# zrc0622/HIRL4UCAV

Measured on AMD Instinct MI355X. Metric: env steps/sec (whole node) + HIRL update steps/sec at 4096 envs/GPU, higher is better.
Workload: dtype f32

## Files before the change

hirl4ucav_amd/csrc/hx_wgrad.hip:

```cpp
#include <cmath>

#include "hx_update.h"

using namespace hxnn;
using namespace hxu;

namespace {

struct WgJobC {
    const float* net; float* grad;
    float* ws0; float* ws1;
    float* mom; float* var; float* target; uint16_t* w2b; float* w2f;
    uint32_t cfg;
    int32_t rows0, rows1;
    float slope, w_given, warm, inv_batch;
    float b1, b2, eps, step_size, bc2_sqrt, tau;
    uint32_t pad_;
    const int* soft_count; float* wstate; float* losses;
    uint16_t* w2tb; uint16_t* tgt_w2b;
    float* count_out;
};
static_assert(sizeof(WgJobC) == 176, "WgJobC layout");
struct WgArgsC {
    WgJobC job[2];
    int has_pre, pre_batch;
    SampleDev pre;
};

struct AdamElem {
    float p, m, v, t;
    __device__ __forceinline__ void fetch(const WgJob& J, unsigned idx) {
        p = J.p[idx];
        m = J.mom[idx];
        v = J.var[idx];
        t = J.target ? J.target[idx] : 0.0f;
    }
    __device__ __forceinline__ void apply(const WgJob& J, const WgAdam& a, unsigned idx, float g) {
        adam_update(p, m, v, g, a.b1, a.b2, a.eps, a.step_size, a.bc2_sqrt);
        J.p[idx] = p;
        J.mom[idx] = m;
        J.var[idx] = v;
        if (J.target) {
            t = polyak_update(t, p, a.tau);
            J.target[idx] = t;
        }
    }
};

constexpr int kWgTilesPerBlock = 2 * (H2 / 16);
constexpr int kWgCols = 16;
constexpr int kWgVecWgs = H2 / kWgCols;
constexpr int kWgL1Wgs = H1 / kWgCols;
constexpr int kWgRG = kWide / kWgCols;
constexpr int kWgPerJob = kWgTilesPerBlock + kWgVecWgs + kWgL1Wgs;
constexpr int kWgRowChunk = 256;

constexpr int kRedP = 21;
__device__ __forceinline__ float sum_groups(const float* p, int half) {
    constexpr int N = kWgRG / 2;
    float v[N];
#pragma unroll
    for (int g = 0; g < N; ++g) v[g] = p[(2 * g + half) * kWgCols * kRedP];
#pragma unroll
    for (int w = 1; w < N; w *= 2)
#pragma unroll
        for (int g = 0; g < N; g += 2 * w) v[g] += v[g + w];
    const float other = __int_as_float(__builtin_amdgcn_mov_dpp(__float_as_int(v[0]), 0xB1, 0xf, 0xf, true));
    return half ? other + v[0] : v[0] + other;
}

__device__ __forceinline__ void expand_wg(const WgJobC& c, WgJob& J, WgArgs& A) {
    J.net = c.net; J.grad = c.grad; J.m = mlp_of(c.cfg & 1023u);
    J.nslots = (int)((c.cfg >> 10) & 3u);
    J.wmode[0] = (int)((c.cfg >> 12) & 3u); J.wmode[1] = (int)((c.cfg >> 14) & 3u);
    J.ws[0] = carve_slot(c.ws0, c.rows0); J.ws[1] = carve_slot(c.ws1, c.rows1);
    J.rows[0] = c.rows0; J.rows[1] = c.rows1;
    J.p = const_cast<float*>(c.net); J.mom = c.mom; J.var = c.var; J.target = c.target; J.w2b = c.w2b; J.w2f = c.w2f;
    J.w2tb = c.w2tb; J.tgt_w2b = c.tgt_w2b; J.w2b_x9 = (int)((c.cfg >> 20) & 1u);
    A.slope = c.slope; A.w_kind = (int)((c.cfg >> 16) & 3u); A.w_given = c.w_given; A.warm = c.warm; A.inv_batch = c.inv_batch;
    A.soft_count = c.soft_count; A.wstate = c.wstate;
    A.ad.b1 = c.b1; A.ad.b2 = c.b2; A.ad.eps = c.eps; A.ad.step_size = c.step_size; A.ad.bc2_sqrt = c.bc2_sqrt; A.ad.tau = c.tau;
    A.ad.finish_actor = (int)((c.cfg >> 18) & 1u); A.ad.use_bc = (int)((c.cfg >> 19) & 1u);
    A.ad.losses = c.losses; A.ad.wstate = c.wstate;
    A.count_out = c.count_out;
    A.ad.alpha_state = nullptr; A.ad.target_entropy = 0.0f; A.ad.alpha_step_size = 0.0f;
    if ((c.cfg >> 21) & 1u) {
        A.ad.alpha_state = c.wstate; A.ad.target_entropy = c.w_given; A.ad.alpha_step_size = c.warm;
        A.ad.wstate = nullptr; A.wstate = nullptr; A.w_given = 0.0f; A.warm = 0.0f;
    }
}
inline WgJobC pack_wg(const WgJob& J, const WgArgs& A) {
    WgJobC c{};
    c.net = J.net; c.grad = J.grad; c.ws0 = J.ws[0].x; c.ws1 = J.nslots > 1 ? J.ws[1].x : J.ws[0].x;
    c.mom = J.mom; c.var = J.var; c.target = J.target; c.w2b = J.w2b; c.w2f = J.w2f; c.w2tb = J.w2tb; c.tgt_w2b = J.tgt_w2b;
    c.cfg = mlp_bits(J.m) | ((uint32_t)J.nslots << 10) | ((uint32_t)J.wmode[0] << 12) | ((uint32_t)J.wmode[1] << 14) | ((uint32_t)A.w_kind << 16) |
            ((uint32_t)(A.ad.finish_actor ? 1 : 0) << 18) | ((uint32_t)(A.ad.use_bc ? 1 : 0) << 19) | ((uint32_t)(J.w2b_x9 ? 1 : 0) << 20) |
            ((uint32_t)(A.ad.alpha_state ? 1 : 0) << 21);
    c.rows0 = J.rows[0]; c.rows1 = J.nslots > 1 ? J.rows[1] : J.rows[0];
    c.slope = A.slope; c.w_given = A.w_given; c.warm = A.warm; c.inv_batch = A.inv_batch;
    c.b1 = A.ad.b1; c.b2 = A.ad.b2; c.eps = A.ad.eps; c.step_size = A.ad.step_size; c.bc2_sqrt = A.ad.bc2_sqrt; c.tau = A.ad.tau;
    c.soft_count = A.soft_count; c.wstate = const_cast<float*>(A.wstate); c.losses = A.ad.losses; c.count_out = A.count_out;
    if (A.ad.alpha_state) { c.wstate = A.ad.alpha_state; c.w_given = A.ad.target_entropy; c.warm = A.ad.alpha_step_size; }
    return c;
}

#ifdef HX_STAMPS_L1
#define STAMP_L1() STAMP()
#else
#define STAMP_L1()
#endif
template <bool ADAM, bool RELU, bool BF16 = false>
__global__ __launch_bounds__(kWide) void wgrad_kernel(WgArgsC AC) {
    __shared__ __attribute__((aligned(16))) float lds[kWgRowChunk * XP + kWgRowChunk * 12 + kWgRG * kWgCols * kRedP];
    float* xs = lds;
    float* rinfo = lds + kWgRowChunk * XP;
    float* red = rinfo + kWgRowChunk * 12;

    {
        static_assert(sizeof(lds) >= (4 * kFusedSlots + 2 * kFusedBatchMax) * 4, "predraw_wg's tables fit");
        if (AC.has_pre && blockIdx.x >= kWgPerJob) {
            if (blockIdx.x == kWgPerJob && blockIdx.y == 0) predraw_wg(AC.pre, AC.pre_batch, lds);
            return;
        }
    }
    const int j = blockIdx.y, b = blockIdx.x;
    WgJob J;
    WgArgs A;
    expand_wg(AC.job[j], J, A);
    const int tid = threadIdx.x, wave = tid >> 6, lane = tid & 63;
    const float slope = A.slope;
    STAMP_DECL;
    STAMP();
    const float w = effective_w(A.w_kind, A.w_given, A.warm, A.inv_batch, A.soft_count, A.wstate);
    float scale[2];
#pragma unroll
    for (int s = 0; s < 2; ++s) scale[s] = J.wmode[s] == 0 ? 1.0f : (J.wmode[s] == 1 ? 1.0f - w : w);
#ifdef HX_STAMPS
    asm volatile("" ::"v"(w));
    STAMP();
#endif
    if (A.count_out && blockIdx.x == 0 && blockIdx.y == 0 && tid == 0) *A.count_out = A.soft_count ? (float)*A.soft_count : 0.0f;
    if (ADAM && A.ad.finish_actor && blockIdx.x == 0 && blockIdx.y == 0 && tid == 0) {
        if (A.ad.use_bc) {
            A.ad.losses[1] = A.ad.losses[2] * w + A.ad.losses[3] * (1.0f - w);
            A.ad.losses[5] = w;
            *A.ad.wstate = w;
        } else {
            A.ad.losses[1] = A.ad.losses[3];
        }
    }
    if (ADAM && A.ad.alpha_state && blockIdx.x == 0 && blockIdx.y == 0 && tid == 0)
        sac_alpha_step(A.ad.alpha_state, A.ad.losses, A.ad.losses[4], A.ad.target_entropy, A.ad.b1, A.ad.b2, A.ad.eps, A.ad.alpha_step_size, A.ad.bc2_sqrt);

    if (b < kWgTilesPerBlock) {
        const int n0 = (b >> 1) * 16, k0 = (b & 1) * (H1 / 2) + (wave & 7) * 16, half = wave >> 3;
        const int r = lane & 15, g = lane >> 4;
        v4f acc = {0.f, 0.f, 0.f, 0.f};
        #pragma unroll
        for (int s = 0; s < 2; ++s) if (s < J.nslots) {
            const float sc = scale[s];
            const float* dz = J.ws[s].dz2;
            const float* h1 = J.ws[s].h1;
            const unsigned dzo = (unsigned)(n0 + r), h1o = (unsigned)(k0 + r);
            const int rows = J.rows[s];
            const int hr = ((rows + 7) >> 3) << 2;
            const int rbeg = half * hr, rend = min(rows, rbeg + hr);
            if constexpr (BF16) {
                v4f accs = {0.f, 0.f, 0.f, 0.f};
                for (int c0 = rbeg; c0 < rend; c0 += 64) {
                    float av[2][8], hv[2][8];
#pragma unroll
                    for (int m = 0; m < 2; ++m)
#pragma unroll
                        for (int j = 0; j < 8; ++j) {
                            const int row = c0 + 32 * m + 8 * g + j;
                            const unsigned rc = (unsigned)(row < rows ? row : rows - 1);
                            av[m][j] = dz[rc * (unsigned)H2 + dzo];
                            hv[m][j] = h1[rc * (unsigned)H1 + h1o];
                        }
#pragma unroll
                    for (int m = 0; m < 2; ++m) {
#pragma unroll
                        for (int j = 0; j < 8; ++j)
                            if (c0 + 32 * m + 8 * g + j >= rend) av[m][j] = 0.0f;
                        accs = mfma16_bf16(pack8_bf16(av[m]), pack8_bf16(hv[m]), accs);
                    }
                }
#pragma unroll
                for (int q = 0; q < 4; ++q) acc[q] = __builtin_fmaf(sc, accs[q], acc[q]);
            } else {
                for (int c0 = rbeg; c0 < rend; c0 += 64) {
                    float av[16], hv[16];
#pragma unroll
                    for (int i = 0; i < 16; ++i) {
                        const int row = c0 + 4 * i + g;
                        const unsigned rc = (unsigned)(row < rows ? row : rows - 1);
                        av[i] = dz[rc * (unsigned)H2 + dzo];
                        hv[i] = h1[rc * (unsigned)H1 + h1o];
                    }
#pragma unroll
                    for (int i = 0; i < 16; ++i) acc = mfma16(av[i] * (c0 + 4 * i + g < rend ? sc : 0.0f), hv[i], acc);
                }
            }
        }
        STAMP();
        const int q0 = 2 * half;
        AdamElem ae[2];
        if (ADAM) {
#pragma unroll
            for (int q = 0; q < 2; ++q) ae[q].fetch(J, J.m.W2() + (n0 + 4 * g + q0 + q) * H1 + k0 + r);
        }
        float2* xch = reinterpret_cast<float2*>(red);
        xch[((wave & 7) * 2 + half) * 64 + lane] = half ? make_float2(acc[0], acc[1]) : make_float2(acc[2], acc[3]);
        __syncthreads();
        const float2 got = xch[((wave & 7) * 2 + (half ^ 1)) * 64 + lane];
        const float fin[2] = {half ? got.x + acc[2] : acc[0] + got.x, half ? got.y + acc[3] : acc[1] + got.y};
        float* out = J.grad + J.m.W2();
#pragma unroll
        for (int q = 0; q < 2; ++q) out[(unsigned)((n0 + 4 * g + q0 + q) * H1 + k0 + r)] = fin[q];
        if (ADAM) {
#pragma unroll
            for (int q = 0; q < 2; ++q) {
                const int idx = J.m.W2() + (n0 + 4 * g + q0 + q) * H1 + k0 + r;
                ae[q].apply(J, A.ad, idx, fin[q]);
                if (J.w2b) {
                    const uint32_t ix = w2_image_index((uint32_t)(n0 + 4 * g + q0 + q), (uint32_t)(k0 + r));
                    uint16_t hi, mid, lo;
                    split3_bf16(ae[q].p, hi, mid, lo);
                    J.w2b[ix] = hi;
                    if (J.w2b_x9) { J.w2b[kImgElems + ix] = mid; J.w2b[2 * kImgElems + ix] = lo; }
                }
                if (J.w2f) J.w2f[w2f_image_index((uint32_t)(n0 + 4 * g + q0 + q), (uint32_t)(k0 + r))] = ae[q].p;
                if (J.w2tb) {
                    const __bf16 bv = (__bf16)ae[q].p;
                    J.w2tb[w2t_image_index((uint32_t)(k0 + r), (uint32_t)(n0 + 4 * g + q0 + q))] = __builtin_bit_cast(uint16_t, bv);
                }
                if (J.target && J.tgt_w2b) {
                    const __bf16 bv = (__bf16)ae[q].t;
                    J.tgt_w2b[w2_image_index((uint32_t)(n0 + 4 * g + q0 + q), (uint32_t)(k0 + r))] = __builtin_bit_cast(uint16_t, bv);
                }
            }
        }
        STAMP();
        STAMP_FLUSH(32, blockIdx.x == 0 && blockIdx.y == 0 && tid == 0);
        SPAN_LOG(HX_SPAN_WGRAD);
        return;
    }
    const int cl = lane & (kWgCols - 1);
    const int rg = tid / kWgCols;
    const int ohalf = tid & 1, oitem = (tid >> 1) / kWgCols, ocol = (tid >> 1) % kWgCols;
    if (b < kWgTilesPerBlock + kWgVecWgs) {
        constexpr int RP = 12;
        const int vb = b - kWgTilesPerBlock;
        const int n = vb * kWgCols + cl;
        const float g2 = J.net[J.m.g2() + n], be2 = J.net[J.m.be2() + n];
        float w3[OW];
#pragma unroll
        for (int jj = 0; jj < OW; ++jj) w3[jj] = jj < J.m.out ? J.net[J.m.W3() + jj * H2 + n] : 0.0f;
        float db2 = 0.f, dg = 0.f, dbe = 0.f, dw3[OW] = {}, db3 = 0.f;
        const int on = vb * kWgCols + ocol;
        const unsigned vidx = (unsigned)(oitem == 0 ? J.m.b2() + on : oitem == 1 ? J.m.g2() + on : oitem == 2 ? J.m.be2() + on : J.m.W3() + (oitem - 3) * H2 + on);
        const bool vlive = oitem < 3 + J.m.out;
        const bool b3live = vb == 0 && oitem == 3 + OW && ocol < J.m.out;
        const unsigned b3idx = (unsigned)(J.m.b3() + (ocol < J.m.out ? ocol : 0));
        AdamElem vae;
        bool vae_pending = ADAM && (vlive || b3live) && ohalf == 0;
        #pragma unroll
        for (int s = 0; s < 2; ++s) if (s < J.nslots) {
            const Slot& S = J.ws[s];
            const float sc = scale[s];
            for (int c0 = 0; c0 < J.rows[s]; c0 += kWgRowChunk) {
                const int nr = min(kWgRowChunk, J.rows[s] - c0);
                float zv[4], dv[4];
#pragma unroll
                for (int i = 0; i < 4; ++i) if (kWgRG * i < nr) {
                    const int r = rg + kWgRG * i;
                    const unsigned o = (unsigned)(c0 + (r < nr ? r : nr - 1)) * (unsigned)H2 + (unsigned)n;
                    zv[i] = S.z2[o];
                    dv[i] = S.dz2[o];
                }
                static_assert(kWgRowChunk <= kWide, "staging: one row per thread");
                const int er = tid < nr ? tid : 0;
                v2f st2v;
                v4f d4, d5;
                if (__builtin_amdgcn_readfirstlane(tid) < nr) {
                    st2v = *reinterpret_cast<const v2f*>(S.st2 + (size_t)(c0 + er) * 2);
                    d4 = *reinterpret_cast<const v4f*>(S.dout + (size_t)(c0 + er) * OW);
                    d5 = *reinterpret_cast<const v4f*>(S.dout + (size_t)(c0 + er) * OW + 4);
                }
                if (vae_pending) {
                    vae.fetch(J, b3live ? b3idx : vidx);
                    vae_pending = false;
                }
                __syncthreads();
                if (tid < nr) {
                    float4* r4 = reinterpret_cast<float4*>(rinfo + tid * RP);
                    r4[0] = make_float4(st2v[0], st2v[1], d4[0], d4[1]);
                    r4[1] = make_float4(d4[2], d4[3], d5[0], d5[1]);
                    r4[2] = make_float4(d5[2], d5[3], 0.0f, 0.0f);
                }
                __syncthreads();
                for (int rb0 = 0; rb0 < nr; rb0 += kWgRG * 4) {
                    const int rb = rg + rb0;
                    if (rb0 != 0) {
#pragma unroll
                        for (int i = 0; i < 4; ++i) if (rb0 + kWgRG * i < nr) {
                            const int r = rb + kWgRG * i;
                            const unsigned o = (unsigned)(c0 + (r < nr ? r : nr - 1)) * (unsigned)H2 + (unsigned)n;
                            zv[i] = S.z2[o];
                            dv[i] = S.dz2[o];
                        }
                    }
#pragma unroll
                    for (int i = 0; i < 4; ++i) {
                        const int r = rb + kWgRG * i;
                        if (r < nr) {
                            float ri[RP];
                            {
                                const float4* r4 = reinterpret_cast<const float4*>(rinfo + r * RP);
                                const float4 a = r4[0], b4 = r4[1], c4 = r4[2];
                                ri[0] = a.x; ri[1] = a.y; ri[2] = a.z; ri[3] = a.w; ri[4] = b4.x; ri[5] = b4.y; ri[6] = b4.z; ri[7] = b4.w;
                                ri[8] = c4.x; ri[9] = c4.y; ri[10] = c4.z; ri[11] = c4.w;
                            }
                            const float xh = (zv[i] - ri[0]) * ri[1];
                            const float y = g2 * xh + be2;
                            float dh2 = (ri[2] * w3[0] + ri[3] * w3[1]) + (ri[4] * w3[2] + ri[5] * w3[3]);
                            if (J.m.out > 4) dh2 += (ri[6] * w3[4] + ri[7] * w3[5]) + (ri[8] * w3[6] + ri[9] * w3[7]);
                            const float dy = act_bwd<RELU>(dh2, y, slope);
                            const float h2 = act_f<RELU>(y, slope);
                            db2 += sc * dv[i];
                            dbe += sc * dy;
                            dg += sc * dy * xh;
#pragma unroll
                            for (int jj = 0; jj < OW; ++jj) dw3[jj] += sc * ri[2 + jj] * h2;
                            if (vb == 0 && cl < J.m.out) db3 += sc * rinfo[r * RP + 2 + cl];
                        }
                    }
                }
            }
        }
        STAMP();
        float* my = red + (rg * kWgCols + cl) * kRedP;
        my[0] = db2; my[1] = dg; my[2] = dbe;
#pragma unroll
        for (int jj = 0; jj < OW; ++jj) my[3 + jj] = dw3[jj];
        my[3 + OW] = db3;
        __syncthreads();
        if (vlive || b3live) {
            float v = sum_groups(red + ocol * kRedP + oitem, ohalf);
            if ((oitem == 1 || oitem == 2) && J.m.no_ln) v = 0.0f;
            const unsigned idx = b3live ? b3idx : vidx;
            if (ohalf == 0) {
                J.grad[idx] = v;
                if (ADAM) vae.apply(J, A.ad, idx, v);
            }
        }
        STAMP();
        STAMP_FLUSH(40, b == kWgTilesPerBlock && j == 0 && tid == 0);
        SPAN_LOG(HX_SPAN_WGRAD);
        return;
    }
    {
        const int kb = (b - kWgTilesPerBlock - kWgVecWgs) * kWgCols;
        const int k = kb + cl;
        const int in = J.m.in;
        const float g1 = J.net[J.m.g1() + k], be1 = J.net[J.m.be1() + k];
        STAMP_L1();
        float db1 = 0.f, dg = 0.f, dbe = 0.f, dw1[17];
#pragma unroll
        for (int i = 0; i < 17; ++i) dw1[i] = 0.f;
        const int ok = kb + ocol;
        const unsigned lidx = (unsigned)(oitem == 0 ? J.m.b1() + ok : oitem == 1 ? J.m.g1() + ok : oitem == 2 ? J.m.be1() + ok : J.m.W1() + ok * in + (oitem - 3));
        const bool llive = oitem < 3 + in;
        AdamElem lae;
        bool lae_pending = ADAM && llive && ohalf == 0;
        #pragma unroll
        for (int s = 0; s < 2; ++s) if (s < J.nslots) {
            const Slot& S = J.ws[s];
            const float sc = scale[s];
            for (int c0 = 0; c0 < J.rows[s]; c0 += kWgRowChunk) {
                const int nr = min(kWgRowChunk, J.rows[s] - c0);
                float zv[4], dv[4];
#pragma unroll
                for (int i = 0; i < 4; ++i) if (kWgRG * i < nr) {
                    const int r = rg + kWgRG * i;
                    const unsigned o = (unsigned)(c0 + (r < nr ? r : nr - 1)) * (unsigned)H1 + (unsigned)k;
                    zv[i] = S.z1[o];
                    dv[i] = S.dh1[o];
                }
                STAMP_L1();
                static_assert(kWgRowChunk * XP <= 5 * kWide && kWgRowChunk <= kWide && kColWgB == 8, "staging: five words + one row per thread");
                const int w0 = __builtin_amdgcn_readfirstlane(tid);
                float xst[5];
#pragma unroll
                for (int q = 0; q < 5; ++q) {
                    const int e = tid + q * kWide;
                    if (w0 + q * kWide < nr * XP) xst[q] = S.x[(size_t)c0 * XP + (e < nr * XP ? e : 0)];
                }
                STAMP_L1();
                const int er = tid < nr ? tid : 0;
                v2f st1v;
                v4f l0, l1, l2, l3;
                if (w0 < nr) {
                    st1v = *reinterpret_cast<const v2f*>(S.st1 + (size_t)(c0 + er) * 2);
                    const v4f* lp4 = reinterpret_cast<const v4f*>(S.lnp + (size_t)(c0 + er) * (2 * kColWgB));
                    l0 = lp4[0]; l1 = lp4[1]; l2 = lp4[2]; l3 = lp4[3];
                }
                STAMP_L1();
                if (lae_pending) {
                    lae.fetch(J, lidx);
                    lae_pending = false;
                }
                STAMP_L1();
                __syncthreads();
                STAMP_L1();
#pragma unroll
                for (int q = 0; q < 5; ++q) {
                    const int e = tid + q * kWide;
                    if (e < nr * XP) xs[e] = xst[q];
                }
                if (tid < nr) {
                    const float s1 = ((l0[0] + l0[2]) + (l1[0] + l1[2])) + ((l2[0] + l2[2]) + (l3[0] + l3[2]));
                    const float s2 = ((l0[1] + l0[3]) + (l1[1] + l1[3])) + ((l2[1] + l2[3]) + (l3[1] + l3[3]));
                    *reinterpret_cast<float4*>(rinfo + tid * 8) = make_float4(st1v[0], st1v[1], s1 * (1.0f / H1), s2 * (1.0f / H1));
                }
                __syncthreads();
                STAMP_L1();
                for (int rb0 = 0; rb0 < nr; rb0 += kWgRG * 4) {
                    const int rb = rg + rb0;
                    if (rb0 != 0) {
#pragma unroll
                        for (int i = 0; i < 4; ++i) if (rb0 + kWgRG * i < nr) {
                            const int r = rb + kWgRG * i;
                            const unsigned o = (unsigned)(c0 + (r < nr ? r : nr - 1)) * (unsigned)H1 + (unsigned)k;
                            zv[i] = S.z1[o];
                            dv[i] = S.dh1[o];
                        }
                    }
#pragma unroll
                    for (int i = 0; i < 4; ++i) {
                        const int r = rb + kWgRG * i;
                        if (r < nr) {
                            const float4 ri = *reinterpret_cast<const float4*>(rinfo + r * 8);
                            const float xh = (zv[i] - ri.x) * ri.y;
                            const float dy = act_bwd<RELU>(dv[i], g1 * xh + be1, slope);
                            const float dz = sc * (ri.y * (dy * g1 - ri.z - xh * ri.w));
                            db1 += dz;
                            dbe += sc * dy;
                            dg += sc * dy * xh;
                            const float4* xr4 = reinterpret_cast<const float4*>(xs + r * XP);
#pragma unroll
                            for (int q = 0; q < 4; ++q) {
                                const float4 x4 = xr4[q];
                                dw1[4 * q] += dz * x4.x; dw1[4 * q + 1] += dz * x4.y; dw1[4 * q + 2] += dz * x4.z; dw1[4 * q + 3] += dz * x4.w;
                            }
                            dw1[16] += dz * xs[r * XP + 16];
                        }
                    }
                }
            }
        }
        STAMP_L1();
        float* my = red + (rg * kWgCols + cl) * kRedP;
        my[0] = db1; my[1] = dg; my[2] = dbe;
#pragma unroll
        for (int i = 0; i < 17; ++i) my[3 + i] = dw1[i];
        STAMP_L1();
        __syncthreads();
        STAMP_L1();
        if (llive) {
            float v = sum_groups(red + ocol * kRedP + oitem, ohalf);
            if ((oitem == 1 || oitem == 2) && J.m.no_ln) v = 0.0f;
#ifdef HX_STAMPS
            asm volatile("" ::"v"(v));
            STAMP_L1();
#endif
            if (ohalf == 0) {
                J.grad[lidx] = v;
                if (ADAM) lae.apply(J, A.ad, lidx, v);
            }
        }
        STAMP_L1();
        STAMP_FLUSH(48, b == kWgTilesPerBlock + kWgVecWgs && j == 0 && tid == 0);
        SPAN_LOG(HX_SPAN_WGRAD);
    }
}

__device__ __forceinline__ float adam_w(const AdamArgs& A) {
    if (A.countf && A.w_kind == 1) {
        const float w = *A.countf * A.inv_batch + A.warm;
        return w > 1.0f ? 1.0f : w;
    }
    return effective_w(A.w_kind, A.w_given, A.warm, A.inv_batch, A.soft_count, A.wstate);
}

__global__ __launch_bounds__(kThreads) void adam_kernel(AdamArgs A) {
    if (A.guard && __hip_atomic_load(A.guard, __ATOMIC_RELAXED, __HIP_MEMORY_SCOPE_SYSTEM) != 0u) return;
    if (A.alpha_state && blockIdx.x == 0 && threadIdx.x == 0)
        sac_alpha_step(A.alpha_state, A.losses, A.losses[4], A.target_entropy, A.b1, A.b2, A.eps, A.alpha_step_size, A.bc2_sqrt);
    const float wmix = A.g2 ? adam_w(A) : 0.0f;
    if (A.finish_actor && blockIdx.x == 0 && threadIdx.x == 0) {
        if (A.use_bc) {
            const float w = adam_w(A);
            A.losses[1] = A.losses[2] * w + A.losses[3] * (1.0f - w);
            A.losses[5] = w;
            *A.wstate = w;
        } else {
            A.losses[1] = A.losses[3];
        }
    }
    const int i = (blockIdx.x * kThreads + threadIdx.x) * 4;
    if (i >= A.n) return;
    if (i + 4 <= A.n) {
        float4 g4 = *reinterpret_cast<const float4*>(A.g + i);
        if (A.g2) {
            const float4 b4 = *reinterpret_cast<const float4*>(A.g2 + i);
            g4.x = wmix * b4.x + (1.0f - wmix) * g4.x;
            g4.y = wmix * b4.y + (1.0f - wmix) * g4.y;
            g4.z = wmix * b4.z + (1.0f - wmix) * g4.z;
            g4.w = wmix * b4.w + (1.0f - wmix) * g4.w;
        }
        adam_step4(A, i, make_float4(g4.x * A.gscale, g4.y * A.gscale, g4.z * A.gscale, g4.w * A.gscale));
        return;
    }
    for (int c = 0; c < A.n - i; ++c) {
        float pv = A.p[i + c], mv = A.m[i + c], vv = A.v[i + c];
        const float gv = A.g2 ? wmix * A.g2[i + c] + (1.0f - wmix) * A.g[i + c] : A.g[i + c];
        adam_update(pv, mv, vv, gv * A.gscale, A.b1, A.b2, A.eps, A.step_size, A.bc2_sqrt);
        A.p[i + c] = pv; A.m[i + c] = mv; A.v[i + c] = vv;
        if (A.target) A.target[i + c] = polyak_update(A.target[i + c], pv, A.tau);
    }
}

__global__ __launch_bounds__(kThreads) void polyak_kernel(float* target, const float* source, int n, float tau, float* target2 = nullptr,
                                                          const float* source2 = nullptr, int n2 = 0, const uint32_t* guard = nullptr) {
    if (guard && *guard != 0u) return;
    const int nb1 = (n / 4 + kThreads) / kThreads;
    int blk = blockIdx.x;
    if (blk >= nb1) {
        blk -= nb1; target = target2; source = source2; n = n2;
    }
    const int i = (blk * kThreads + threadIdx.x) * 4;
    if (i >= n) return;
    if (i + 4 <= n) {
        float4 t4 = *reinterpret_cast<const float4*>(target + i);
        const float4 s4 = *reinterpret_cast<const float4*>(source + i);
        t4.x = polyak_update(t4.x, s4.x, tau);
        t4.y = polyak_update(t4.y, s4.y, tau);
        t4.z = polyak_update(t4.z, s4.z, tau);
        t4.w = polyak_update(t4.w, s4.w, tau);
        *reinterpret_cast<float4*>(target + i) = t4;
        return;
    }
    for (int c = 0; c < n - i; ++c) target[i + c] = polyak_update(target[i + c], source[i + c], tau);
}

}

namespace hxu {

void launch_wg(const WgArgs& W, bool adam, hipStream_t st) {
    WgArgsC C{};
    for (int j = 0; j < W.njobs; ++j) C.job[j] = pack_wg(W.job[j], W);
    const bool pre = W.predraw != nullptr;
    C.has_pre = pre ? 1 : 0;
    if (pre) { C.pre = *W.predraw; C.pre_batch = W.predraw_batch; }
    const dim3 grid(kWgPerJob + (pre ? 8 : 0), W.njobs);
    const bool relu = W.slope == 0.0f;
#define HX_WG(ADAM_, RELU_, BF16_) hipLaunchKernelGGL((wgrad_kernel<ADAM_, RELU_, BF16_>), grid, dim3(kWide), 0, st, C)
    static const int dbg_off = getenv("HX_DBG_BF16_OFF") ? atoi(getenv("HX_DBG_BF16_OFF")) : 0;
    if (W.bf16 && !(dbg_off & 4)) {
        if (adam) { if (relu) HX_WG(true, true, true); else HX_WG(true, false, true); }
        else { if (relu) HX_WG(false, true, true); else HX_WG(false, false, true); }
    } else {
        if (adam) { if (relu) HX_WG(true, true, false); else HX_WG(true, false, false); }
        else { if (relu) HX_WG(false, true, false); else HX_WG(false, false, false); }
    }
#undef HX_WG
}
void launch_adam(const AdamArgs& A, hipStream_t st) {
    hipLaunchKernelGGL(adam_kernel, dim3((A.n / 4 + kThreads) / kThreads), dim3(kThreads), 0, st, A);
}
void launch_polyak(float* target, const float* source, int n, float tau, float* target2, const float* source2, int n2, hipStream_t st, const uint32_t* guard) {
    const int nb = (n / 4 + kThreads) / kThreads + (target2 ? (n2 / 4 + kThreads) / kThreads : 0);
    hipLaunchKernelGGL(polyak_kernel, dim3(nb), dim3(kThreads), 0, st, target, source, n, tau, target2, source2, n2, guard);
}

}

extern "C" {

static int adam_impl(const HxNets* N, const HxHyper* Hy, int32_t which, int32_t step, float grad_scale, int32_t w_kind, float w_given,
                     float warm, int32_t batch, const float* msg, void* stream) {
    const bool polyak = (which & 16) != 0;
    which &= 15;
    HX_REQUIRE(N && Hy && step >= 1 && which >= 0 && which <= 2, "hx_adam: bad arguments");
    AdamArgs A{};
    A.n = which == 0 ? 2 * kQ.padded() : kActor.size();
    A.p = which == 0 ? N->critic : N->actor;
    A.g = which == 0 ? N->grad_critic : N->grad_actor;
    A.m = which == 0 ? N->m_critic : N->m_actor;
    A.v = which == 0 ? N->v_critic : N->v_actor;
    set_adam_scalars(A, which == 0 ? Hy->lr_critic : Hy->lr_actor, step);
    A.gscale = grad_scale;
    A.finish_actor = which == 1;
    A.w_kind = w_kind; A.w_given = w_given; A.warm = warm; A.inv_batch = 1.0f / (batch > 0 ? batch : 1);
    A.soft_count = N->soft_count; A.wstate = N->wstate; A.losses = N->losses; A.use_bc = Hy->use_bc;
    if (polyak) {
        A.target = which == 0 ? N->target_critic : N->target_actor;
        A.tau = Hy->tau;
    }
    if (which != 0 && N->actor_w2_f32i) {
        A.w2f = N->actor_w2_f32i;
        A.w2_lo = kActor.W2();
    }
    if (which != 0 && N->actor_w2_bf16 && !N->w2_bf16_all) {
        A.w2b = N->actor_w2_bf16;
        A.w2_lo = kActor.W2();
    }
    if (which != 0 && N->actor_w2_x9) {
        HX_REQUIRE(!N->actor_w2_bf16 && !N->w2_bf16_all, "hx_adam: actor_w2_x9 excludes the plain bf16 images (one acting format at a time)");
        A.w2b = N->actor_w2_x9;
        A.w2b_x9 = 1;
        A.w2_lo = kActor.W2();
    }
    if (uint16_t* im = N->w2_bf16_all) {
        HX_REQUIRE(!N->actor_w2_bf16 || N->actor_w2_bf16 == im + IM_ACTOR * kImgElems, "hx_adam: with w2_bf16_all set, actor_w2_bf16 must be NULL or its first image");
        if (which == 0) {
            A.nseg = 2;
            for (int h = 0; h < 2; ++h) {
                A.seg_lo[h] = h * kQ.padded() + kQ.W2();
                A.seg_w2b[h] = im + (IM_C1 + h) * kImgElems;
                A.seg_w2tb[h] = im + (IM_C1_T + h) * kImgElems;
                A.seg_tgt_w2b[h] = im + (IM_TC1 + h) * kImgElems;
            }
        } else {
            A.nseg = 1;
            A.seg_lo[0] = kActor.W2();
            A.seg_w2b[0] = im + IM_ACTOR * kImgElems;
            A.seg_w2tb[0] = im + IM_ACTOR_T * kImgElems;
            A.seg_tgt_w2b[0] = im + IM_TA * kImgElems;
        }
    }
    A.guard = N->xchg_status;
    if (msg) {
        HX_REQUIRE(which == 1 && (reinterpret_cast<uintptr_t>(msg) & 15u) == 0, "hx_adam_mixed: actor step only, 16-byte aligned message");
        A.g = msg;
        if (Hy->use_bc) {
            A.g2 = msg + kActor.padded();
            A.countf = msg + 2 * kActor.padded();
        }
    }
    HX_REQUIRE((((uintptr_t)A.p | (uintptr_t)A.g | (uintptr_t)A.m | (uintptr_t)A.v) & 15u) == 0, "hx_adam: buffers must be 16-byte aligned");
    launch_adam(A, (hipStream_t)stream);
    HX_CHECK_LAUNCH("hx_adam");
    return 0;
}
int hx_adam(const HxNets* N, const HxHyper* Hy, int32_t which, int32_t step, float grad_scale, int32_t w_kind, float w_given,
            float warm, int32_t batch, void* stream) {
    return adam_impl(N, Hy, which, step, grad_scale, w_kind, w_given, warm, batch, nullptr, stream);
}
int hx_adam_mixed(const HxNets* N, const HxHyper* Hy, int32_t polyak, int32_t step, float grad_scale, int32_t w_kind, float w_given,
                  float warm, int32_t batch, const float* msg, void* stream) {
    HX_REQUIRE(msg, "hx_adam_mixed: null message");
    return adam_impl(N, Hy, 1 | (polyak ? 16 : 0), step, grad_scale, w_kind, w_given, warm, batch, msg, stream);
}

int hx_polyak(const HxNets* N, const HxHyper* Hy, void* stream) {
    HX_REQUIRE(N && Hy, "hx_polyak: bad arguments");
    const int nc = 2 * kQ.padded(), na = kActor.size();
    launch_polyak(N->target_critic, N->critic, nc, Hy->tau, N->target_actor, N->actor, na, (hipStream_t)stream, N->xchg_status);
    if (uint16_t* im = N->w2_bf16_all) {
        launch_pack_bf16(N->target_actor + kActor.W2(), im + IM_TA * kImgElems, false, (hipStream_t)stream);
        for (int h = 0; h < 2; ++h)
            launch_pack_bf16(N->target_critic + h * kQ.padded() + kQ.W2(), im + (IM_TC1 + h) * kImgElems, false, (hipStream_t)stream);
    }
    HX_CHECK_LAUNCH("hx_polyak");
    return 0;
}

int hx_sac_adam(const HxSacNets* N, const HxHyper* Hy, int32_t which, int32_t step, float grad_scale, float target_entropy, void* stream) {
    HX_REQUIRE(N && Hy && step >= 1 && (which == 0 || which == 1), "hx_sac_adam: bad arguments");
    AdamArgs A{};
    if (int rc = sac_adam_fill(A, N, Hy, which, step, grad_scale, target_entropy, true, "hx_sac_adam")) return rc;
    launch_adam(A, (hipStream_t)stream);
    HX_CHECK_LAUNCH("hx_sac_adam");
    return 0;
}

}

HX_DEFINE_DEBUG_COLLECTORS(wgrad, 32, 56)
```

Baseline: 79.54 million.

## Add two-slot weight-gradient kernel that splits work across twice as many workgroups

Adds a wgrad2 kernel for the single-job, two-slot case with small row counts. It uses half-width column tiles, so the grid has twice as many workgroups, and each block splits its rows into two stages whose partial sums are handed off through LDS. The goal is to fill more compute units when only one job (e.g. actor) runs, which the old kernel left underused. The kernel and existing bodies are refactored into shared helper functions. The cost is extra barriers and duplicated staging, and the path can be turned off with HX_WGRAD_TWO_SLOT=0.

```diff
diff --git a/hirl4ucav_amd/csrc/hx_wgrad.hip b/hirl4ucav_amd/csrc/hx_wgrad.hip
--- a/hirl4ucav_amd/csrc/hx_wgrad.hip
+++ b/hirl4ucav_amd/csrc/hx_wgrad.hip
@@ -56,11 +56,12 @@
 constexpr int kWgRowChunk = 256;
 
 constexpr int kRedP = 21;
+template <int COLS = kWgCols>
 __device__ __forceinline__ float sum_groups(const float* p, int half) {
     constexpr int N = kWgRG / 2;
     float v[N];
 #pragma unroll
-    for (int g = 0; g < N; ++g) v[g] = p[(2 * g + half) * kWgCols * kRedP];
+    for (int g = 0; g < N; ++g) v[g] = p[(2 * g + half) * COLS * kRedP];
 #pragma unroll
     for (int w = 1; w < N; w *= 2)
 #pragma unroll
@@ -104,6 +105,123 @@
     return c;
 }
 
+template <bool ADAM>
+__device__ __forceinline__ void wg_thread0(const WgArgs& A, float w) {
+    if (A.count_out) *A.count_out = A.soft_count ? (float)*A.soft_count : 0.0f;
+    if (ADAM && A.ad.finish_actor) {
+        if (A.ad.use_bc) {
+            A.ad.losses[1] = A.ad.losses[2] * w + A.ad.losses[3] * (1.0f - w);
+            A.ad.losses[5] = w;
+            *A.ad.wstate = w;
+        } else {
+            A.ad.losses[1] = A.ad.losses[3];
+        }
+    }
+    if (ADAM && A.ad.alpha_state)
+        sac_alpha_step(A.ad.alpha_state, A.ad.losses, A.ad.losses[4], A.ad.target_entropy, A.ad.b1, A.ad.b2, A.ad.eps, A.ad.alpha_step_size, A.ad.bc2_sqrt);
+}
+__device__ __forceinline__ void tile_load(const float* dz, const float* h1, unsigned dzo, unsigned h1o, int c0, int g, int rows, float (&av)[16], float (&hv)[16]) {
+#pragma unroll
+    for (int i = 0; i < 16; ++i) {
+        const int row = c0 + 4 * i + g;
+        const unsigned rc = (unsigned)(row < rows ? row : rows - 1);
+        av[i] = dz[rc * (unsigned)H2 + dzo];
+        hv[i] = h1[rc * (unsigned)H1 + h1o];
+    }
+}
+__device__ __forceinline__ void tile_mfma(const float (&av)[16], const float (&hv)[16], int c0, int g, int rend, float sc, v4f& acc) {
+#pragma unroll
+    for (int i = 0; i < 16; ++i) acc = mfma16(av[i] * (c0 + 4 * i + g < rend ? sc : 0.0f), hv[i], acc);
+}
+template <bool ADAM>
+__device__ __forceinline__ void tile_finish(const WgJob& J, const WgAdam& ad, const v4f acc, int n0, int k0, int r, int g, int half, int pair, bool live,
+                                            float2* xch, int lane) {
+    const int q0 = 2 * half;
+    AdamElem ae[2];
+    if (ADAM && live) {
+#pragma unroll
+        for (int q = 0; q < 2; ++q) ae[q].fetch(J, J.m.W2() + (n0 + 4 * g + q0 + q) * H1 + k0 + r);
+    }
+    if (live) xch[(pair * 2 + half) * 64 + lane] = half ? make_float2(acc[0], acc[1]) : make_float2(acc[2], acc[3]);
+    __syncthreads();
+    if (!live) return;
+    const float2 got = xch[(pair * 2 + (half ^ 1)) * 64 + lane];
+    const float fin[2] = {half ? got.x + acc[2] : acc[0] + got.x, half ? got.y + acc[3] : acc[1] + got.y};
+    float* out = J.grad + J.m.W2();
+#pragma unroll
+    for (int q = 0; q < 2; ++q) out[(unsigned)((n0 + 4 * g + q0 + q) * H1 + k0 + r)] = fin[q];
+    if (ADAM) {
+#pragma unroll
+        for (int q = 0; q < 2; ++q) {
+            const int idx = J.m.W2() + (n0 + 4 * g + q0 + q) * H1 + k0 + r;
+            ae[q].apply(J, ad, idx, fin[q]);
+            if (J.w2b) {
+                const uint32_t ix = w2_image_index((uint32_t)(n0 + 4 * g + q0 + q), (uint32_t)(k0 + r));
+                uint16_t hi, mid, lo;
+                split3_bf16(ae[q].p, hi, mid, lo);
+                J.w2b[ix] = hi;
+                if (J.w2b_x9) { J.w2b[kImgElems + ix] = mid; J.w2b[2 * kImgElems + ix] = lo; }
+            }
+            if (J.w2f) J.w2f[w2f_image_index((uint32_t)(n0 + 4 * g + q0 + q), (uint32_t)(k0 + r))] = ae[q].p;
+            if (J.w2tb) {
+                const __bf16 bv = (__bf16)ae[q].p;
+                J.w2tb[w2t_image_index((uint32_t)(k0 + r), (uint32_t)(n0 + 4 * g + q0 + q))] = __builtin_bit_cast(uint16_t, bv);
+            }
+            if (J.target && J.tgt_w2b) {
+                const __bf16 bv = (__bf16)ae[q].t;
+                J.tgt_w2b[w2_image_index((uint32_t)(n0 + 4 * g + q0 + q), (uint32_t)(k0 + r))] = __builtin_bit_cast(uint16_t, bv);
+            }
+        }
+    }
+}
+struct VecAcc {
+    float db2, dg, dbe, dw3[OW], db3;
+};
+constexpr int kVecRP = 12;
+template <bool RELU>
+__device__ __forceinline__ void vec_row(VecAcc& a, const float* rrow, float z, float d, float g2, float be2, const float (&w3)[OW], int out, float slope, float sc,
+                                        bool b3col, int cl) {
+    float ri[kVecRP];
+    {
+        const float4* r4 = reinterpret_cast<const float4*>(rrow);
+        const float4 a4 = r4[0], b4 = r4[1], c4 = r4[2];
+        ri[0] = a4.x; ri[1] = a4.y; ri[2] = a4.z; ri[3] = a4.w; ri[4] = b4.x; ri[5] = b4.y; ri[6] = b4.z; ri[7] = b4.w;
+        ri[8] = c4.x; ri[9] = c4.y; ri[10] = c4.z; ri[11] = c4.w;
+    }
+    const float xh = (z - ri[0]) * ri[1];
+    const float y = g2 * xh + be2;
+    float dh2 = (ri[2] * w3[0] + ri[3] * w3[1]) + (ri[4] * w3[2] + ri[5] * w3[3]);
+    if (out > 4) dh2 += (ri[6] * w3[4] + ri[7] * w3[5]) + (ri[8] * w3[6] + ri[9] * w3[7]);
+    const float dy = act_bwd<RELU>(dh2, y, slope);
+    const float h2 = act_f<RELU>(y, slope);
+    a.db2 += sc * d;
+    a.dbe += sc * dy;
+    a.dg += sc * dy * xh;
+#pragma unroll
+    for (int jj = 0; jj < OW; ++jj) a.dw3[jj] += sc * ri[2 + jj] * h2;
+    if (b3col) a.db3 += sc * rrow[2 + cl];
+}
+struct L1Acc {
+    float db1, dg, dbe, dw1[17];
+};
+template <bool RELU>
+__device__ __forceinline__ void l1_row(L1Acc& a, const float* rrow, const float* xrow, float z, float d, float g1, float be1, float slope, float sc) {
+    const float4 ri = *reinterpret_cast<const float4*>(rrow);
+    const float xh = (z - ri.x) * ri.y;
+    const float dy = act_bwd<RELU>(d, g1 * xh + be1, slope);
+    const float dz = sc * (ri.y * (dy * g1 - ri.z - xh * ri.w));
+    a.db1 += dz;
+    a.dbe += sc * dy;
+    a.dg += sc * dy * xh;
+    const float4* xr4 = reinterpret_cast<const float4*>(xrow);
+#pragma unroll
+    for (int q = 0; q < 4; ++q) {
+        const float4 x4 = xr4[q];
+        a.dw1[4 * q] += dz * x4.x; a.dw1[4 * q + 1] += dz * x4.y; a.dw1[4 * q + 2] += dz * x4.z; a.dw1[4 * q + 3] += dz * x4.w;
+    }
+    a.dw1[16] += dz * xrow[16];
+}
+
 #ifdef HX_STAMPS_L1
 #define STAMP_L1() STAMP()
 #else
@@ -139,18 +257,7 @@
     asm volatile("" ::"v"(w));
     STAMP();
 #endif
-    if (A.count_out && blockIdx.x == 0 && blockIdx.y == 0 && tid == 0) *A.count_out = A.soft_count ? (float)*A.soft_count : 0.0f;
-    if (ADAM && A.ad.finish_actor && blockIdx.x == 0 && blockIdx.y == 0 && tid == 0) {
-        if (A.ad.use_bc) {
-            A.ad.losses[1] = A.ad.losses[2] * w + A.ad.losses[3] * (1.0f - w);
-            A.ad.losses[5] = w;
-            *A.ad.wstate = w;
-        } else {
-            A.ad.losses[1] = A.ad.losses[3];
-        }
-    }
-    if (ADAM && A.ad.alpha_state && blockIdx.x == 0 && blockIdx.y == 0 && tid == 0)
-        sac_alpha_step(A.ad.alpha_state, A.ad.losses, A.ad.losses[4], A.ad.target_entropy, A.ad.b1, A.ad.b2, A.ad.eps, A.ad.alpha_step_size, A.ad.bc2_sqrt);
+    if (blockIdx.x == 0 && blockIdx.y == 0 && tid == 0) wg_thread0<ADAM>(A, w);
 
     if (b < kWgTilesPerBlock) {
         const int n0 = (b >> 1) * 16, k0 = (b & 1) * (H1 / 2) + (wave & 7) * 16, half = wave >> 3;
@@ -191,56 +298,13 @@
             } else {
                 for (int c0 = rbeg; c0 < rend; c0 += 64) {
                     float av[16], hv[16];
-#pragma unroll
-                    for (int i = 0; i < 16; ++i) {
-                        const int row = c0 + 4 * i + g;
-                        const unsigned rc = (unsigned)(row < rows ? row : rows - 1);
-                        av[i] = dz[rc * (unsigned)H2 + dzo];
-                        hv[i] = h1[rc * (unsigned)H1 + h1o];
-                    }
-#pragma unroll
-                    for (int i = 0; i < 16; ++i) acc = mfma16(av[i] * (c0 + 4 * i + g < rend ? sc : 0.0f), hv[i], acc);
+                    tile_load(dz, h1, dzo, h1o, c0, g, rows, av, hv);
+                    tile_mfma(av, hv, c0, g, rend, sc, acc);
                 }
             }
         }
         STAMP();
-        const int q0 = 2 * half;
-        AdamElem ae[2];
-        if (ADAM) {
-#pragma unroll
-            for (int q = 0; q < 2; ++q) ae[q].fetch(J, J.m.W2() + (n0 + 4 * g + q0 + q) * H1 + k0 + r);
-        }
-        float2* xch = reinterpret_cast<float2*>(red);
-        xch[((wave & 7) * 2 + half) * 64 + lane] = half ? make_float2(acc[0], acc[1]) : make_float2(acc[2], acc[3]);
-        __syncthreads();
-        const float2 got = xch[((wave & 7) * 2 + (half ^ 1)) * 64 + lane];
-        const float fin[2] = {half ? got.x + acc[2] : acc[0] + got.x, half ? got.y + acc[3] : acc[1] + got.y};
-        float* out = J.grad + J.m.W2();
-#pragma unroll
-        for (int q = 0; q < 2; ++q) out[(unsigned)((n0 + 4 * g + q0 + q) * H1 + k0 + r)] = fin[q];
-        if (ADAM) {
-#pragma unroll
-            for (int q = 0; q < 2; ++q) {
-                const int idx = J.m.W2() + (n0 + 4 * g + q0 + q) * H1 + k0 + r;
-                ae[q].apply(J, A.ad, idx, fin[q]);
-                if (J.w2b) {
-                    const uint32_t ix = w2_image_index((uint32_t)(n0 + 4 * g + q0 + q), (uint32_t)(k0 + r));
-                    uint16_t hi, mid, lo;
-                    split3_bf16(ae[q].p, hi, mid, lo);
-                    J.w2b[ix] = hi;
-                    if (J.w2b_x9) { J.w2b[kImgElems + ix] = mid; J.w2b[2 * kImgElems + ix] = lo; }
-                }
-                if (J.w2f) J.w2f[w2f_image_index((uint32_t)(n0 + 4 * g + q0 + q), (uint32_t)(k0 + r))] = ae[q].p;
-                if (J.w2tb) {
-                    const __bf16 bv = (__bf16)ae[q].p;
-                    J.w2tb[w2t_image_index((uint32_t)(k0 + r), (uint32_t)(n0 + 4 * g + q0 + q))] = __builtin_bit_cast(uint16_t, bv);
-                }
-                if (J.target && J.tgt_w2b) {
-                    const __bf16 bv = (__bf16)ae[q].t;
-                    J.tgt_w2b[w2_image_index((uint32_t)(n0 + 4 * g + q0 + q), (uint32_t)(k0 + r))] = __builtin_bit_cast(uint16_t, bv);
-                }
-            }
-        }
+        tile_finish<ADAM>(J, A.ad, acc, n0, k0, r, g, half, wave & 7, true, reinterpret_cast<float2*>(red), lane);
         STAMP();
         STAMP_FLUSH(32, blockIdx.x == 0 && blockIdx.y == 0 && tid == 0);
         SPAN_LOG(HX_SPAN_WGRAD);
@@ -250,14 +314,14 @@
     const int rg = tid / kWgCols;
     const int ohalf = tid & 1, oitem = (tid >> 1) / kWgCols, ocol = (tid >> 1) % kWgCols;
     if (b < kWgTilesPerBlock + kWgVecWgs) {
-        constexpr int RP = 12;
+        constexpr int RP = kVecRP;
         const int vb = b - kWgTilesPerBlock;
         const int n = vb * kWgCols + cl;
         const float g2 = J.net[J.m.g2() + n], be2 = J.net[J.m.be2() + n];
         float w3[OW];
 #pragma unroll
         for (int jj = 0; jj < OW; ++jj) w3[jj] = jj < J.m.out ? J.net[J.m.W3() + jj * H2 + n] : 0.0f;
-        float db2 = 0.f, dg = 0.f, dbe = 0.f, dw3[OW] = {}, db3 = 0.f;
+        VecAcc a = {};
         const int on = vb * kWgCols + ocol;
         const unsigned vidx = (unsigned)(oitem == 0 ? J.m.b2() + on : oitem == 1 ? J.m.g2() + on : oitem == 2 ? J.m.be2() + on : J.m.W3() + (oitem - 3) * H2 + on);
         const bool vlive = oitem < 3 + J.m.out;
@@ -314,37 +378,17 @@
 #pragma unroll
                     for (int i = 0; i < 4; ++i) {
                         const int r = rb + kWgRG * i;
-                        if (r < nr) {
-                            float ri[RP];
-                            {
-                                const float4* r4 = reinterpret_cast<const float4*>(rinfo + r * RP);
-                                const float4 a = r4[0], b4 = r4[1], c4 = r4[2];
-                                ri[0] = a.x; ri[1] = a.y; ri[2] = a.z; ri[3] = a.w; ri[4] = b4.x; ri[5] = b4.y; ri[6] = b4.z; ri[7] = b4.w;
-                                ri[8] = c4.x; ri[9] = c4.y; ri[10] = c4.z; ri[11] = c4.w;
-                            }
-                            const float xh = (zv[i] - ri[0]) * ri[1];
-                            const float y = g2 * xh + be2;
-                            float dh2 = (ri[2] * w3[0] + ri[3] * w3[1]) + (ri[4] * w3[2] + ri[5] * w3[3]);
-                            if (J.m.out > 4) dh2 += (ri[6] * w3[4] + ri[7] * w3[5]) + (ri[8] * w3[6] + ri[9] * w3[7]);
-                            const float dy = act_bwd<RELU>(dh2, y, slope);
-                            const float h2 = act_f<RELU>(y, slope);
-                            db2 += sc * dv[i];
-                            dbe += sc * dy;
-                            dg += sc * dy * xh;
-#pragma unroll
-                            for (int jj = 0; jj < OW; ++jj) dw3[jj] += sc * ri[2 + jj] * h2;
-                            if (vb == 0 && cl < J.m.out) db3 += sc * rinfo[r * RP + 2 + cl];
-                        }
+                        if (r < nr) vec_row<RELU>(a, rinfo + r * RP, zv[i], dv[i], g2, be2, w3, J.m.out, slope, sc, vb == 0 && cl < J.m.out, cl);
                     }
                 }
             }
         }
         STAMP();
         float* my = red + (rg * kWgCols + cl) * kRedP;
-        my[0] = db2; my[1] = dg; my[2] = dbe;
-#pragma unroll
-        for (int jj = 0; jj < OW; ++jj) my[3 + jj] = dw3[jj];
-        my[3 + OW] = db3;
+        my[0] = a.db2; my[1] = a.dg; my[2] = a.dbe;
+#pragma unroll
+        for (int jj = 0; jj < OW; ++jj) my[3 + jj] = a.dw3[jj];
+        my[3 + OW] = a.db3;
         __syncthreads();
         if (vlive || b3live) {
             float v = sum_groups(red + ocol * kRedP + oitem, ohalf);
@@ -366,9 +410,7 @@
         const int in = J.m.in;
         const float g1 = J.net[J.m.g1() + k], be1 = J.net[J.m.be1() + k];
         STAMP_L1();
-        float db1 = 0.f, dg = 0.f, dbe = 0.f, dw1[17];
-#pragma unroll
-        for (int i = 0; i < 17; ++i) dw1[i] = 0.f;
+        L1Acc a = {};
         const int ok = kb + ocol;
         const unsigned lidx = (unsigned)(oitem == 0 ? J.m.b1() + ok : oitem == 1 ? J.m.g1() + ok : oitem == 2 ? J.m.be1() + ok : J.m.W1() + ok * in + (oitem - 3));
         const bool llive = oitem < 3 + in;
@@ -440,31 +482,16 @@
 #pragma unroll
                     for (int i = 0; i < 4; ++i) {
                         const int r = rb + kWgRG * i;
-                        if (r < nr) {
-                            const float4 ri = *reinterpret_cast<const float4*>(rinfo + r * 8);
-                            const float xh = (zv[i] - ri.x) * ri.y;
-                            const float dy = act_bwd<RELU>(dv[i], g1 * xh + be1, slope);
-                            const float dz = sc * (ri.y * (dy * g1 - ri.z - xh * ri.w));
-                            db1 += dz;
-                            dbe += sc * dy;
-                            dg += sc * dy * xh;
-                            const float4* xr4 = reinterpret_cast<const float4*>(xs + r * XP);
-#pragma unroll
-                            for (int q = 0; q < 4; ++q) {
-                                const float4 x4 = xr4[q];
-                                dw1[4 * q] += dz * x4.x; dw1[4 * q + 1] += dz * x4.y; dw1[4 * q + 2] += dz * x4.z; dw1[4 * q + 3] += dz * x4.w;
-                            }
-                            dw1[16] += dz * xs[r * XP + 16];
-                        }
+                        if (r < nr) l1_row<RELU>(a, rinfo + r * 8, xs + r * XP, zv[i], dv[i], g1, be1, slope, sc);
                     }
                 }
             }
         }
         STAMP_L1();
         float* my = red + (rg * kWgCols + cl) * kRedP;
-        my[0] = db1; my[1] = dg; my[2] = dbe;
-#pragma unroll
-        for (int i = 0; i < 17; ++i) my[3 + i] = dw1[i];
+        my[0] = a.db1; my[1] = a.dg; my[2] = a.dbe;
+#pragma unroll
+        for (int i = 0; i < 17; ++i) my[3 + i] = a.dw1[i];
         STAMP_L1();
         __syncthreads();
         STAMP_L1();
@@ -486,6 +513,256 @@
     }
 }
 
+constexpr int kWg2Cols = kWgCols / 2;
+constexpr int kWg2Tiles = 4 * (H2 / 16);
+constexpr int kWg2VecWgs = H2 / kWg2Cols;
+constexpr int kWg2L1Wgs = H1 / kWg2Cols;
+constexpr int kWg2PerJob = kWg2Tiles + kWg2VecWgs + kWg2L1Wgs;
+static_assert(kWide / 2 / kWg2Cols == kWgRG && kWg2PerJob == 2 * kWgPerJob, "two stages of 64 row groups; as many workgroups as the critics' two jobs");
+template <bool ADAM, bool RELU>
+__global__ __launch_bounds__(kWide) void wgrad2_kernel(WgArgsC AC) {
+    __shared__ __attribute__((aligned(16))) float lds[kWgRowChunk * XP + kWgRowChunk * 12 + kWgRG * kWgCols * kRedP];
+    float* xs = lds;
+    float* rinfo = lds + kWgRowChunk * XP;
+    float* red = rinfo + kWgRowChunk * 12;
+    float* hand = red + kWgRG * kWg2Cols * kRedP;
+    static_assert((kWgRG * kWg2Cols * kRedP) % 4 == 0 && 8 * 64 * 4 <= kWgRG * kWg2Cols * kRedP, "the tile hand-off is 16-byte aligned and fits");
+
+    if (AC.has_pre && blockIdx.x >= kWg2PerJob) {
+        if (blockIdx.x == kWg2PerJob) predraw_wg(AC.pre, AC.pre_batch, lds);
+        return;
+    }
+    const int b = blockIdx.x;
+    WgJob J;
+    WgArgs A;
+    expand_wg(AC.job[0], J, A);
+    const int tid = threadIdx.x, wave = tid >> 6, lane = tid & 63;
+    const int stage = __builtin_amdgcn_readfirstlane(tid) >> 9;
+    const float slope = A.slope;
+    STAMP_DECL;
+    STAMP();
+    const float w = effective_w(A.w_kind, A.w_given, A.warm, A.inv_batch, A.soft_count, A.wstate);
+    float scale[2];
+#pragma unroll
+    for (int s = 0; s < 2; ++s) scale[s] = J.wmode[s] == 0 ? 1.0f : (J.wmode[s] == 1 ? 1.0f - w : w);
+    if (blockIdx.x == 0 && tid == 0) wg_thread0<ADAM>(A, w);
+    const float sc = stage ? scale[1] : scale[0];
+    const int rows0 = J.rows[0], rows1 = J.rows[1], nrt = rows0 + rows1;
+    const int nr = stage ? rows1 : rows0, roff = stage ? rows0 : 0;
+
+    if (b < kWg2Tiles) {
+        const int tile = wave & 3, half = (wave >> 2) & 1;
+        const int n0 = (b >> 2) * 16, k0 = (b & 3) * (H1 / 4) + tile * 16;
+        const int r = lane & 15, g = lane >> 4;
+        const float* dz = stage ? J.ws[1].dz2 : J.ws[0].dz2;
+        const float* h1 = stage ? J.ws[1].h1 : J.ws[0].h1;
+        const unsigned dzo = (unsigned)(n0 + r), h1o = (unsigned)(k0 + r);
+        const int hr = ((nr + 7) >> 3) << 2;
+        const int rbeg = half * hr, rend = min(nr, rbeg + hr);
+        float av[16], hv[16];
+        if (rbeg < rend) tile_load(dz, h1, dzo, h1o, rbeg, g, nr, av, hv);
+        v4f acc = {0.f, 0.f, 0.f, 0.f};
+        v4f* hnd = reinterpret_cast<v4f*>(hand) + (tile * 2 + half) * 64 + lane;
+        if (stage == 0) {
+            for (int c0 = rbeg; c0 < rend; c0 += 64) {
+                if (c0 != rbeg) tile_load(dz, h1, dzo, h1o, c0, g, nr, av, hv);
+                tile_mfma(av, hv, c0, g, rend, sc, acc);
+            }
+            *hnd = acc;
+        }
+        __syncthreads();
+        if (stage == 1) {
+            acc = *hnd;
+            for (int c0 = rbeg; c0 < rend; c0 += 64) {
+                if (c0 != rbeg) tile_load(dz, h1, dzo, h1o, c0, g, nr, av, hv);
+                tile_mfma(av, hv, c0, g, rend, sc, acc);
+            }
+        }
+        tile_finish<ADAM>(J, A.ad, acc, n0, k0, r, g, half, tile, stage == 1, reinterpret_cast<float2*>(red), lane);
+        SPAN_LOG(HX_SPAN_WGRAD);
+        return;
+    }
+    const int cl = lane & (kWg2Cols - 1);
+    const int rg = (tid & (kWide / 2 - 1)) / kWg2Cols;
+    const int ohalf = tid & 1, oitem = (tid >> 1) / kWg2Cols, ocol = (tid >> 1) % kWg2Cols;
+    const int w0 = __builtin_amdgcn_readfirstlane(tid);
+    const bool mine0 = tid < rows0;
+    const int er = tid < nrt ? (mine0 ? tid : tid - rows0) : 0;
+    float* hnd = hand + (rg * kWg2Cols + cl) * kRedP;
+    float* my = red + (rg * kWg2Cols + cl) * kRedP;
+    if (b < kWg2Tiles + kWg2VecWgs) {
+        constexpr int RP = kVecRP;
+        const int vb = b - kWg2Tiles;
+        const int n = vb * kWg2Cols + cl;
+        const float g2 = J.net[J.m.g2() + n], be2 = J.net[J.m.be2() + n];
+        float w3[OW];
+#pragma unroll
+        for (int jj = 0; jj < OW; ++jj) w3[jj] = jj < J.m.out ? J.net[J.m.W3() + jj * H2 + n] : 0.0f;
+        static_assert(OW <= kWg2Cols, "db3's columns are in the first column block");
+        const int on = vb * kWg2Cols + ocol;
+        const unsigned vidx = (unsigned)(oitem == 0 ? J.m.b2() + on : oitem == 1 ? J.m.g2() + on : oitem == 2 ? J.m.be2() + on : J.m.W3() + (oitem - 3) * H2 + on);
+        const bool vlive = oitem < 3 + J.m.out;
+        const bool b3live = vb == 0 && oitem == 3 + OW && ocol < J.m.out;
+        const unsigned b3idx = (unsigned)(J.m.b3() + (ocol < J.m.out ? ocol : 0));
+        const float* z2 = stage ? J.ws[1].z2 : J.ws[0].z2;
+        const float* dz2 = stage ? J.ws[1].dz2 : J.ws[0].dz2;
+        float zv[4], dv[4];
+#pragma unroll
+        for (int i = 0; i < 4; ++i) if (kWgRG * i < nr) {
+            const int r = rg + kWgRG * i;
+            const unsigned o = (unsigned)(r < nr ? r : nr - 1) * (unsigned)H2 + (unsigned)n;
+            zv[i] = z2[o];
+            dv[i] = dz2[o];
+        }
+        v2f st2v;
+        v4f d4, d5;
+        if (w0 < nrt) {
+            const float* st2 = mine0 ? J.ws[0].st2 : J.ws[1].st2;
+            const float* dout = mine0 ? J.ws[0].dout : J.ws[1].dout;
+            st2v = *reinterpret_cast<const v2f*>(st2 + (size_t)er * 2);
+            d4 = *reinterpret_cast<const v4f*>(dout + (size_t)er * OW);
+            d5 = *reinterpret_cast<const v4f*>(dout + (size_t)er * OW + 4);
+        }
+        AdamElem vae;
+        if (ADAM && (vlive || b3live) && ohalf == 0) vae.fetch(J, b3live ? b3idx : vidx);
+        if (tid < nrt) {
+            float4* r4 = reinterpret_cast<float4*>(rinfo + tid * RP);
+            r4[0] = make_float4(st2v[0], st2v[1], d4[0], d4[1]);
+            r4[1] = make_float4(d4[2], d4[3], d5[0], d5[1]);
+            r4[2] = make_float4(d5[2], d5[3], 0.0f, 0.0f);
+        }
+        __syncthreads();
+        VecAcc a = {};
+        const bool b3col = vb == 0 && cl < J.m.out;
+        if (stage == 0) {
+#pragma unroll
+            for (int i = 0; i < 4; ++i) {
+                const int r = rg + kWgRG * i;
+                if (r < nr) vec_row<RELU>(a, rinfo + (roff + r) * RP, zv[i], dv[i], g2, be2, w3, J.m.out, slope, sc, b3col, cl);
+            }
+            hnd[0] = a.db2; hnd[1] = a.dg; hnd[2] = a.dbe;
+#pragma unroll
+            for (int jj = 0; jj < OW; ++jj) hnd[3 + jj] = a.dw3[jj];
+            hnd[3 + OW] = a.db3;
+        }
+        __syncthreads();
+        if (stage == 1) {
+            a.db2 = hnd[0]; a.dg = hnd[1]; a.dbe = hnd[2];
+#pragma unroll
+            for (int jj = 0; jj < OW; ++jj) a.dw3[jj] = hnd[3 + jj];
+            a.db3 = hnd[3 + OW];
+#pragma unroll
+            for (int i = 0; i < 4; ++i) {
+                const int r = rg + kWgRG * i;
+                if (r < nr) vec_row<RELU>(a, rinfo + (roff + r) * RP, zv[i], dv[i], g2, be2, w3, J.m.out, slope, sc, b3col, cl);
+            }
+            my[0] = a.db2; my[1] = a.dg; my[2] = a.dbe;
+#pragma unroll
+            for (int jj = 0; jj < OW; ++jj) my[3 + jj] = a.dw3[jj];
+            my[3 + OW] = a.db3;
+        }
+        __syncthreads();
+        if (vlive || b3live) {
+            float v = sum_groups<kWg2Cols>(red + ocol * kRedP + oitem, ohalf);
+            if ((oitem == 1 || oitem == 2) && J.m.no_ln) v = 0.0f;
+            const unsigned idx = b3live ? b3idx : vidx;
+            if (ohalf == 0) {
+                J.grad[idx] = v;
+                if (ADAM) vae.apply(J, A.ad, idx, v);
+            }
+        }
+        SPAN_LOG(HX_SPAN_WGRAD);
+        return;
+    }
+    {
+        const int kb = (b - kWg2Tiles - kWg2VecWgs) * kWg2Cols;
+        const int k = kb + cl;
+        const int in = J.m.in;
+        const float g1 = J.net[J.m.g1() + k], be1 = J.net[J.m.be1() + k];
+        const int ok = kb + ocol;
+        const unsigned lidx = (unsigned)(oitem == 0 ? J.m.b1() + ok : oitem == 1 ? J.m.g1() + ok : oitem == 2 ? J.m.be1() + ok : J.m.W1() + ok * in + (oitem - 3));
+        const bool llive = oitem < 3 + in;
+        const float* z1 = stage ? J.ws[1].z1 : J.ws[0].z1;
+        const float* dh1 = stage ? J.ws[1].dh1 : J.ws[0].dh1;
+        float zv[4], dv[4];
+#pragma unroll
+        for (int i = 0; i < 4; ++i) if (kWgRG * i < nr) {
+            const int r = rg + kWgRG * i;
+            const unsigned o = (unsigned)(r < nr ? r : nr - 1) * (unsigned)H1 + (unsigned)k;
+            zv[i] = z1[o];
+            dv[i] = dh1[o];
+        }
+        static_assert(kWgRowChunk * XP <= 5 * kWide && kWgRowChunk <= kWide && kColWgB == 8, "staging: five words + one row per thread");
+        const int nx0 = rows0 * XP, nxt = nrt * XP;
+        float xst[5];
+#pragma unroll
+        for (int q = 0; q < 5; ++q) {
+            const int e = tid + q * kWide;
+            if (w0 + q * kWide < nxt) {
+                const float* xp = e < nx0 ? J.ws[0].x : J.ws[1].x;
+                xst[q] = xp[e < nxt ? (e < nx0 ? e : e - nx0) : 0];
+            }
+        }
+        v2f st1v;
+        v4f l0, l1, l2, l3;
+        if (w0 < nrt) {
+            const float* st1 = mine0 ? J.ws[0].st1 : J.ws[1].st1;
+            const float* lnp = mine0 ? J.ws[0].lnp : J.ws[1].lnp;
+            st1v = *reinterpret_cast<const v2f*>(st1 + (size_t)er * 2);
+            const v4f* lp4 = reinterpret_cast<const v4f*>(lnp + (size_t)er * (2 * kColWgB));
+            l0 = lp4[0]; l1 = lp4[1]; l2 = lp4[2]; l3 = lp4[3];
+        }
+        AdamElem lae;
+        if (ADAM && llive && ohalf == 0) lae.fetch(J, lidx);
+#pragma unroll
+        for (int q = 0; q < 5; ++q) {
+            const int e = tid + q * kWide;
+            if (e < nxt) xs[e] = xst[q];
+        }
+        if (tid < nrt) {
+            const float s1 = ((l0[0] + l0[2]) + (l1[0] + l1[2])) + ((l2[0] + l2[2]) + (l3[0] + l3[2]));
+            const float s2 = ((l0[1] + l0[3]) + (l1[1] + l1[3])) + ((l2[1] + l2[3]) + (l3[1] + l3[3]));
+            *reinterpret_cast<float4*>(rinfo + tid * 8) = make_float4(st1v[0], st1v[1], s1 * (1.0f / H1), s2 * (1.0f / H1));
+        }
+        __syncthreads();
+        L1Acc a = {};
+        if (stage == 0) {
+#pragma unroll
+            for (int i = 0; i < 4; ++i) {
+                const int r = rg + kWgRG * i;
+                if (r < nr) l1_row<RELU>(a, rinfo + (roff + r) * 8, xs + (roff + r) * XP, zv[i], dv[i], g1, be1, slope, sc);
+            }
+            hnd[0] = a.db1; hnd[1] = a.dg; hnd[2] = a.dbe;
+#pragma unroll
+            for (int i = 0; i < 17; ++i) hnd[3 + i] = a.dw1[i];
+        }
+        __syncthreads();
+        if (stage == 1) {
+            a.db1 = hnd[0]; a.dg = hnd[1]; a.dbe = hnd[2];
+#pragma unroll
+            for (int i = 0; i < 17; ++i) a.dw1[i] = hnd[3 + i];
+#pragma unroll
+            for (int i = 0; i < 4; ++i) {
+                const int r = rg + kWgRG * i;
+                if (r < nr) l1_row<RELU>(a, rinfo + (roff + r) * 8, xs + (roff + r) * XP, zv[i], dv[i], g1, be1, slope, sc);
+            }
+            my[0] = a.db1; my[1] = a.dg; my[2] = a.dbe;
+#pragma unroll
+            for (int i = 0; i < 17; ++i) my[3 + i] = a.dw1[i];
+        }
+        __syncthreads();
+        if (llive) {
+            float v = sum_groups<kWg2Cols>(red + ocol * kRedP + oitem, ohalf);
+            if ((oitem == 1 || oitem == 2) && J.m.no_ln) v = 0.0f;
+            if (ohalf == 0) {
+                J.grad[lidx] = v;
+                if (ADAM) lae.apply(J, A.ad, lidx, v);
+            }
+        }
+        SPAN_LOG(HX_SPAN_WGRAD);
+    }
+}
+
 __device__ __forceinline__ float adam_w(const AdamArgs& A) {
     if (A.countf && A.w_kind == 1) {
         const float w = *A.countf * A.inv_batch + A.warm;
@@ -569,9 +846,17 @@
     const bool relu = W.slope == 0.0f;
 #define HX_WG(ADAM_, RELU_, BF16_) hipLaunchKernelGGL((wgrad_kernel<ADAM_, RELU_, BF16_>), grid, dim3(kWide), 0, st, C)
     static const int dbg_off = getenv("HX_DBG_BF16_OFF") ? atoi(getenv("HX_DBG_BF16_OFF")) : 0;
+    static const bool two_on = !(getenv("HX_WGRAD_TWO_SLOT") && atoi(getenv("HX_WGRAD_TWO_SLOT")) == 0);
+    const WgJob& J0 = W.job[0];
     if (W.bf16 && !(dbg_off & 4)) {
         if (adam) { if (relu) HX_WG(true, true, true); else HX_WG(true, false, true); }
         else { if (relu) HX_WG(false, true, true); else HX_WG(false, false, true); }
+    } else if (two_on && W.njobs == 1 && J0.nslots == 2 && J0.rows[0] > 0 && J0.rows[1] > 0 && J0.rows[0] + J0.rows[1] <= kWgRowChunk) {
+        const dim3 grid2(kWg2PerJob + (pre ? 8 : 0), 1);
+#define HX_WG2(ADAM_, RELU_) hipLaunchKernelGGL((wgrad2_kernel<ADAM_, RELU_>), grid2, dim3(kWide), 0, st, C)
+        if (adam) { if (relu) HX_WG2(true, true); else HX_WG2(true, false); }
+        else { if (relu) HX_WG2(false, true); else HX_WG2(false, false); }
+#undef HX_WG2
     } else {
         if (adam) { if (relu) HX_WG(true, true, false); else HX_WG(true, false, false); }
         else { if (relu) HX_WG(false, true, false); else HX_WG(false, false, false); }
```

Measured after the change: 81.03 million, median of 6. 1.9% higher.
